# AwsGeek/thinvids

Measured on AMD Instinct MI355X. Metric: encoded frames/sec (whole node) at fixed PSNR, 1080p & 4K HEVC, 1/2/4/8 MI355X, higher is better.
Workload: dtype uint8 video / int32 integer transforms (bit-exact HEVC)

## Files before the change

csrc/core/capi.cpp:

```cpp
#include <cstring>
#include <exception>
#include <memory>
#include <string>
#include <vector>

#include "tv/av1_enc.h"
#include "tv/container.h"
#include "tv/cpu_encoder.h"
#include "tv/hevc_codec.h"
#include "tv/me_model.h"
#include "tv/sdh.h"
#include "tv/synth.h"
#include "tv/tb_frag.h"

using namespace tv;

namespace {
thread_local std::string g_err;
template <class F> int guard(F&& f) {
  try {
    f();
    return 0;
  } catch (const std::exception& e) {
    g_err = e.what();
    return -1;
  }
}
struct Bytes {
  std::vector<uint8_t> v;
};
}

extern "C" {

const char* tv_last_error() { return g_err.c_str(); }
int tv_core_version() { return 1; }

void* tv_bytes_new() { return new Bytes(); }
void tv_bytes_free(void* b) { delete static_cast<Bytes*>(b); }
size_t tv_bytes_size(void* b) { return static_cast<Bytes*>(b)->v.size(); }
const uint8_t* tv_bytes_data(void* b) { return static_cast<Bytes*>(b)->v.data(); }
void tv_bytes_clear(void* b) { static_cast<Bytes*>(b)->v.clear(); }

void tv_synth_frame(uint32_t seed, int t, int W, int H, uint8_t* y, uint8_t* u, uint8_t* v) {
  SynthFrameCtx ctx;
  synth_frame_ctx(seed, t, W, H, ctx);
  for (int c = 0; c < 3; ++c) {
    uint8_t* P = c == 0 ? y : (c == 1 ? u : v);
    const int w = c ? W / 2 : W, h = c ? H / 2 : H;
    for (int j = 0; j < h; ++j)
      for (int i = 0; i < w; ++i) P[(size_t)j * w + i] = (uint8_t)synth_sample_ctx(ctx, c, i, j);
  }
}

int tv_satd8x8(const int* d, int stride) { return satd8x8(d, stride); }

void* tv_cpu_encoder_new(int width, int height, int qp, int deblock, int range, int max_merge) {
  SeqConfig cfg;
  cfg.width = width;
  cfg.height = height;
  cfg.qp = qp;
  cfg.set_flags(deblock);
  cfg.max_merge_cand = max_merge;
  cfg.finalize();
  CpuEncoder* e = nullptr;
  guard([&] { e = new CpuEncoder(cfg, range); });
  return e;
}
void* tv_cpu_encoder_new_b(int width, int height, int qp, int deblock, int range, int max_merge, int mgop) {
  SeqConfig cfg;
  cfg.width = width;
  cfg.height = height;
  cfg.qp = qp;
  cfg.set_flags(deblock);
  cfg.max_merge_cand = max_merge;
  cfg.mgop = mgop;
  cfg.finalize();
  CpuEncoder* e = nullptr;
  guard([&] { e = new CpuEncoder(cfg, range); });
  return e;
}
int tv_cpu_encoder_begin_gop(void* e, int nframes, int* disp) {
  return guard([&] {
    auto* enc = static_cast<CpuEncoder*>(e);
    enc->begin_gop(nframes);
    for (size_t k = 0; k < enc->plan().pics.size(); ++k) disp[k] = enc->plan().pics[k].disp;
  });
}
int tv_gop_plan(int nframes, int mgop, int* disp, int* type, int* ref0, int* ref1, int* layer, int* info) {
  const GopPlan g = plan_gop(nframes, mgop);
  for (size_t k = 0; k < g.pics.size(); ++k) {
    disp[k] = g.pics[k].disp;
    type[k] = g.pics[k].type;
    ref0[k] = g.pics[k].ref[0];
    ref1[k] = g.pics[k].ref[1];
    layer[k] = g.pics[k].layer;
  }
  info[0] = g.dpb_size;
  info[1] = g.num_reorder;
  return (int)g.pics.size();
}
void* tv_cpu_encoder_new_crf(int width, int height, int qp, int deblock, int range, int max_merge, int crf) {
  SeqConfig cfg;
  cfg.width = width;
  cfg.height = height;
  cfg.qp = qp;
  cfg.set_flags(deblock);
  cfg.max_merge_cand = max_merge;
  cfg.crf = crf;
  cfg.finalize();
  CpuEncoder* e = nullptr;
  guard([&] { e = new CpuEncoder(cfg, range); });
  return e;
}
void tv_cpu_encoder_free(void* e) { delete static_cast<CpuEncoder*>(e); }
int tv_cpu_encoder_encode(void* e, const uint8_t* y, const uint8_t* u, const uint8_t* v, int sy,
                          int sc, int idr, int poc, void* out) {
  return guard([&] {
    const uint8_t* planes[3] = {y, u, v};
    const int strides[3] = {sy, sc, sc};
    static_cast<CpuEncoder*>(e)->encode_frame(planes, strides, idr != 0, poc, static_cast<Bytes*>(out)->v);
  });
}
int tv_cpu_encoder_encode_qp(void* e, const uint8_t* y, const uint8_t* u, const uint8_t* v, int sy, int sc, int idr,
                             int poc, int qp, void* out) {
  return guard([&] {
    const uint8_t* planes[3] = {y, u, v};
    const int strides[3] = {sy, sc, sc};
    static_cast<CpuEncoder*>(e)->encode_frame(planes, strides, idr != 0, poc, static_cast<Bytes*>(out)->v, qp);
  });
}
void tv_cpu_encoder_recon(void* e, uint8_t* y, uint8_t* u, uint8_t* v) {
  const Picture& p = static_cast<CpuEncoder*>(e)->recon();
  std::memcpy(y, p.y.data(), p.y.size());
// ... 201 lines not shown
```

csrc/gpu/k_frame.hip:

```cpp
#include <cstring>

#include "gpu_common.h"
#include "k_encode.h"
#include "tv/synth.h"

namespace tv {
namespace gpu {

struct VNoiseRow {
  int sh, sy;
  int32_t cy, cx;
  uint32_t seed;
  int a, b, c, d;
  __device__ void init(int32_t py16, int lp, uint32_t sd) {
    sh = lp + 4;
    seed = sd;
    cy = py16 >> sh;
    const int fy = (int)((py16 - (cy << sh)) << 8 >> sh);
    sy = (fy * fy * (768 - 2 * fy)) >> 16;
    cx = INT32_MIN;
  }
  __device__ int eval(int32_t px16) {
    const int32_t nx = px16 >> sh;
    if (nx != cx) {
      if (nx == cx + 1) {
        a = b;
        c = d;
      } else {
        a = synth_hash(nx, cy, seed) & 255;
        c = synth_hash(nx, cy + 1, seed) & 255;
      }
      b = synth_hash(nx + 1, cy, seed) & 255;
      d = synth_hash(nx + 1, cy + 1, seed) & 255;
      cx = nx;
    }
    const int fx = (int)((px16 - (cx << sh)) << 8 >> sh);
    const int sx = (fx * fx * (768 - 2 * fx)) >> 16;
    const int top = a * 256 + (b - a) * sx;
    const int bot = c * 256 + (d - c) * sx;
    return (top * 256 + (bot - top) * sy) >> 16;
  }
};

__device__ __forceinline__ int synth_objects(const SynthFrameCtx& f, int c, int xl, int yl, int v, unsigned rows) {
  for (; rows; rows &= rows - 1) {
    const int k = __builtin_ctz(rows);
    const SynthObject& o = f.obj[k];
    const int32_t rx16 = xl * 16 - f.ox[k], ry16 = yl * 16 - f.oy[k];
    if (rx16 < 0 || rx16 >= o.w * 16) continue;
    if (o.shape == 1) {
      const int64_t dx = 2 * (int64_t)rx16 - o.w * 16, dy = 2 * (int64_t)ry16 - o.h * 16;
      const int64_t ww = (int64_t)o.w * 16, hh = (int64_t)o.h * 16;
      if (dx * dx * hh * hh + dy * dy * ww * ww > ww * ww * hh * hh) continue;
    }
    if (c == 0) {
      v = 40 + ((synth_vnoise(rx16, ry16, 4, o.seed) * 3 + synth_vnoise(rx16, ry16, 2, o.seed + 5)) >> 2) * 3 / 4;
    } else {
      v = 64 + (int)(synth_hash(k, c, f.seed) & 127) + (synth_vnoise(rx16, ry16, 5, o.seed + c) >> 3);
    }
  }
  return v;
}

template <bool kTex>
__global__ void __launch_bounds__(256) k_synth(FrameSet src, Geo g, uint32_t seed, FrameIdx fi) {
  const int c = blockIdx.y, b = blockIdx.z;
  const int pw = c ? g.W / 2 : g.W, ph = c ? g.H / 2 : g.H;
  const int dw = c ? g.dw / 2 : g.dw, dh = c ? g.dh / 2 : g.dh;
  __shared__ SynthFrameCtx ctx;
  if (threadIdx.x == 0) synth_frame_ctx(seed, fi.t[b], g.dw, g.dh, ctx);
  __syncthreads();
  uint8_t* P = src.plane(c, b, g);
  const int s = c ? 1 : 0, pq = pw >> 2;
  constexpr bool tex = kTex;
  for (int i = blockIdx.x * blockDim.x + threadIdx.x; i < pq * ph; i += gridDim.x * blockDim.x) {
    const int y = i / pq, x0 = (i - y * pq) * 4;
    const int yc = tv_min(y, dh - 1), yl = yc << s;
    const int32_t by16 = yl * 16 + ctx.t * (tex ? 36 : 12);
    unsigned rows = 0;
#pragma unroll
    for (int k = 0; k < kSynthObjects; ++k) {
      const int32_t ry16 = yl * 16 - ctx.oy[k];
      rows |= (ry16 >= 0 && ry16 < ctx.obj[k].h * 16) ? 1u << k : 0u;
    }
    VNoiseRow n0, n1, n2, n3;
    if (c == 0) {
      n0.init(by16, 7, ctx.seed);
      n1.init(by16, 5, ctx.seed + 1);
      n2.init(by16, 3, ctx.seed + 2);
      if (tex) n3.init(by16, 1, ctx.seed + 3);
    } else {
      n0.init(by16, 8, ctx.seed + 10 * c);
    }
    uint32_t word = 0;
#pragma unroll
    for (int j = 0; j < 4; ++j) {
      const int xc = tv_min(x0 + j, dw - 1), xl = xc << s;
      const int32_t bx16 = xl * 16 + ctx.t * (tex ? 88 : 36);
      int v;
      if (c == 0 && tex)
        v = (n0.eval(bx16) * 3 + n1.eval(bx16) * 2 + n2.eval(bx16) * 2 + n3.eval(bx16)) >> 3;
      else if (c == 0)
        v = (n0.eval(bx16) * 5 + n1.eval(bx16) * 2 + n2.eval(bx16)) >> 3;
      else
        v = 96 + (n0.eval(bx16) >> 1);
      if (rows) v = synth_objects(ctx, c, xl, yl, v, rows);
      if (tex) {
        const uint32_t gr = synth_hash(xc + ctx.t * 7919, yc + c * 104729, ctx.seed ^ 0x5bd1e995u);
        v += c ? (int)(gr & 3) - 2 : (int)(gr & 7) - 4;
      }
      word |= (uint32_t)clip_pixel(v) << (8 * j);
    }
    *reinterpret_cast<uint32_t*>(P + (long)y * pw + x0) = word;
  }
}

__global__ void __launch_bounds__(256) k_sse(FrameSet a, FrameSet r, Geo g, unsigned long long* sse) {
  const int c = blockIdx.y, b = blockIdx.z;
  const int pw = c ? g.W / 2 : g.W;
  const int dw = c ? g.dw / 2 : g.dw, dh = c ? g.dh / 2 : g.dh;
  const uint8_t* A = a.plane(c, b, g);
  const uint8_t* R = r.plane(c, b, g);
  const int wq = (dw + 3) >> 2;
  unsigned s = 0;
  for (int i = blockIdx.x * blockDim.x + threadIdx.x; i < wq * dh; i += gridDim.x * blockDim.x) {
    const int y = i / wq, x = (i - y * wq) * 4;
    const uint32_t va = *reinterpret_cast<const uint32_t*>(A + (long)y * pw + x);
    const uint32_t vr = *reinterpret_cast<const uint32_t*>(R + (long)y * pw + x);
#pragma unroll
    for (int k = 0; k < 4; ++k) {
      const int d = (int)((va >> (8 * k)) & 255) - (int)((vr >> (8 * k)) & 255);
      s += (x + k < dw) ? (unsigned)(d * d) : 0u;
    }
  }
  unsigned long long t = s;
  for (int o = 32; o > 0; o >>= 1) t += __shfl_xor(t, o, 64);
  __shared__ unsigned long long part[4];
  if ((threadIdx.x & 63) == 0) part[threadIdx.x >> 6] = t;
  __syncthreads();
  if (threadIdx.x == 0) atomicAdd(sse + b * 3 + c, part[0] + part[1] + part[2] + part[3]);
}

typedef short tv_short2 __attribute__((ext_vector_type(2)));

__device__ constexpr uint32_t pack_taps4(int f, int k0) {
  return (uint32_t)(uint8_t)kLumaFilter[f][k0] | (uint32_t)(uint8_t)kLumaFilter[f][k0 + 1] << 8 |
         (uint32_t)(uint8_t)kLumaFilter[f][k0 + 2] << 16 | (uint32_t)(uint8_t)kLumaFilter[f][k0 + 3] << 24;
}
__device__ constexpr uint32_t pack_taps2(int f, int k0) {
  return (uint32_t)(uint16_t)kLumaFilter[f][k0] | (uint32_t)(uint16_t)kLumaFilter[f][k0 + 1] << 16;
}
__device__ __forceinline__ int dot4(uint32_t a, uint32_t b, int c) {
  return __builtin_amdgcn_sdot4((int)a, (int)b, c, false);
}
__device__ __forceinline__ int dot2(uint32_t a, uint32_t b, int c) {
  return __builtin_amdgcn_sdot2(__builtin_bit_cast(tv_short2, a), __builtin_bit_cast(tv_short2, b), c, false);
}
__device__ __forceinline__ uint32_t pack4_pixels(int v0, int v1, int v2, int v3) {
  return (uint32_t)clip_pixel(v0) | (uint32_t)clip_pixel(v1) << 8 | (uint32_t)clip_pixel(v2) << 16 |
         (uint32_t)clip_pixel(v3) << 24;
}

constexpr int kPhW = 10;
__global__ void __launch_bounds__(256) k_phase_planes(FrameSet ref, uint8_t* phase, Geo g) {
  const int tid = threadIdx.x;
  const int L = xcd_remap(blockIdx.x + gridDim.x * (blockIdx.y + gridDim.y * blockIdx.z),
                          gridDim.x * gridDim.y * gridDim.z);
  const int tpf = gridDim.x * gridDim.y, b = L / tpf, tyi = (L - b * tpf) / gridDim.x;
  const int tx0 = (L - b * tpf - tyi * gridDim.x) * 32 - 8, ty0 = tyi * 32 - 8;
  const uint8_t* R = ref.plane(0, b, g);
  __shared__ uint32_t raw[39][kPhW];
  __shared__ __align__(16) int16_t hf[3][39][32];
  for (int i = tid; i < 39 * kPhW; i += 256) {
    const int rr = i / kPhW, w = i - rr * kPhW;
    const uint8_t* row = R + (long)clip3(0, g.H - 1, ty0 - 3 + rr) * g.W;
    const int x = tx0 - 4 + 4 * w;
    uint32_t v;
    if (x >= 0 && x + 3 < g.W) {
      v = *reinterpret_cast<const uint32_t*>(row + x);
    } else {
      v = 0;
#pragma unroll
      for (int k = 0; k < 4; ++k) v |= (uint32_t)row[clip3(0, g.W - 1, x + k)] << (8 * k);
    }
    raw[rr][w] = v ^ 0x80808080u;
  }
  __syncthreads();
  for (int i = tid; i < 39 * 8; i += 256) {
    const int rr = i >> 3, c4 = i & 7;
    const uint32_t w0 = raw[rr][c4], w1 = raw[rr][c4 + 1], w2 = raw[rr][c4 + 2];
    int out[3][4];
#pragma unroll
    for (int j = 0; j < 4; ++j) {
      const uint32_t lo = j == 3 ? w1 : __builtin_amdgcn_alignbyte(w1, w0, j + 1);
      const uint32_t hi = j == 3 ? w2 : __builtin_amdgcn_alignbyte(w2, w1, j + 1);
#pragma unroll
      for (int f = 1; f < 4; ++f) out[f - 1][j] = dot4(lo, pack_taps4(f, 0), dot4(hi, pack_taps4(f, 4), 8192));
// ... 88 lines not shown
  uint8_t* U = rec.plane(1, b, g);
  uint8_t* V = rec.plane(2, b, g);
  const int W = g.W, H = g.H, Wc = W / 2;
  const int qpc = chroma_qp(qp, 0);
  const int nl = horizontal ? (H / 8 - 1) * (W / 4) : (W / 8 - 1) * (H / 4);
  const int nc = horizontal ? (H / 16 - 1) * (Wc / 4) : (W / 16 - 1) * (H / 8);
  auto ld = [](const uint8_t* p) { return *reinterpret_cast<const uint32_t*>(p); };
  auto st = [](uint8_t* p, uint32_t v) { *reinterpret_cast<uint32_t*>(p) = v; };
  for (int i = blockIdx.x * blockDim.x + threadIdx.x; i < nl + nc; i += gridDim.x * blockDim.x) {
    if (i < nl) {
      if (!horizontal) {
        const int x = 8 * (1 + i % (W / 8 - 1)), y = 4 * (i / (W / 8 - 1));
        const int bs = deblock_edge_bs(cl, in, cb, mv, g.w8, x - 1, y, x, y, dir, mv1, tu);
        if (bs) {
          uint32_t v[4][2];
#pragma unroll
          for (int k = 0; k < 4; ++k) {
            v[k][0] = ld(Y + (long)(y + k) * W + x - 4);
            v[k][1] = ld(Y + (long)(y + k) * W + x);
          }
          deblock_luma_edge4(reinterpret_cast<uint8_t*>(&v[0][1]), 1, 8, bs, qp);
#pragma unroll
          for (int k = 0; k < 4; ++k) {
            st(Y + (long)(y + k) * W + x - 4, v[k][0]);
            st(Y + (long)(y + k) * W + x, v[k][1]);
          }
        }
      } else {
        const int y = 8 * (1 + i % (H / 8 - 1)), x = 4 * (i / (H / 8 - 1));
        const int bs = deblock_edge_bs(cl, in, cb, mv, g.w8, x, y - 1, x, y, dir, mv1, tu);
        if (bs) {
          uint32_t v[8];
#pragma unroll
          for (int r = 0; r < 8; ++r) v[r] = ld(Y + (long)(y - 4 + r) * W + x);
          deblock_luma_edge4(reinterpret_cast<uint8_t*>(&v[4]), 4, 1, bs, qp);
#pragma unroll
          for (int r = 1; r < 7; ++r) st(Y + (long)(y - 4 + r) * W + x, v[r]);
        }
      }
    } else {
      const int j = i - nl;
      if (!horizontal) {
        const int xc = 8 * (1 + j % (W / 16 - 1)), yc = 4 * (j / (W / 16 - 1));
        const int bs = deblock_edge_bs(cl, in, cb, mv, g.w8, 2 * xc - 1, 2 * yc, 2 * xc, 2 * yc, dir, mv1, tu);
        if (bs == 2) {
#pragma unroll
          for (int pl = 0; pl < 2; ++pl) {
            uint8_t* P = pl ? V : U;
            uint32_t v[4][2];
#pragma unroll
            for (int k = 0; k < 4; ++k) {
              v[k][0] = ld(P + (long)(yc + k) * Wc + xc - 4);
              v[k][1] = ld(P + (long)(yc + k) * Wc + xc);
            }
            deblock_chroma_edge(reinterpret_cast<uint8_t*>(&v[0][1]), 1, 8, 4, qpc);
#pragma unroll
            for (int k = 0; k < 4; ++k) {
              st(P + (long)(yc + k) * Wc + xc - 4, v[k][0]);
              st(P + (long)(yc + k) * Wc + xc, v[k][1]);
            }
          }
        }
      } else {
        const int yc = 8 * (1 + j % (H / 16 - 1)), xc = 4 * (j / (H / 16 - 1));
        const int bs = deblock_edge_bs(cl, in, cb, mv, g.w8, 2 * xc, 2 * yc - 1, 2 * xc, 2 * yc, dir, mv1, tu);
        if (bs == 2) {
#pragma unroll
          for (int pl = 0; pl < 2; ++pl) {
            uint8_t* P = pl ? V : U;
            uint32_t v[4];
#pragma unroll
            for (int r = 0; r < 4; ++r) v[r] = ld(P + (long)(yc - 2 + r) * Wc + xc);
            deblock_chroma_edge(reinterpret_cast<uint8_t*>(&v[2]), 4, 1, 4, qpc);
            st(P + (long)(yc - 1) * Wc + xc, v[1]);
            st(P + (long)yc * Wc + xc, v[2]);
          }
        }
      }
    }
  }
}

void launch_synth(FrameSet src, const Geo& g, uint32_t seed, const FrameIdx& fi, int B, hipStream_t s) {
  dim3 grid((unsigned)tv_min(512, (int)((g.ysz + 1023) / 1024)), 3, B);
  if (synth_textured(seed))
    k_synth<true><<<grid, 256, 0, s>>>(src, g, seed, fi);
  else
    k_synth<false><<<grid, 256, 0, s>>>(src, g, seed, fi);
}
__global__ void __launch_bounds__(256) k_gather_frames(const uint8_t* frames, long seg_stride, FrameSet src, Geo g,
                                                       int B) {
  const long f16 = (g.ysz + 2 * g.csz) / 16, y16 = g.ysz / 16, c16 = g.csz / 16;
  for (long i = (long)blockIdx.x * 256 + threadIdx.x; i < B * f16; i += (long)gridDim.x * 256) {
    const int b = (int)(i / f16);
    const long r = i - b * f16;
    const uint4 v = reinterpret_cast<const uint4*>(frames + b * seg_stride)[r];
    uint4* d = r < y16 ? reinterpret_cast<uint4*>(src.y + b * g.ysz) + r
               : r < y16 + c16 ? reinterpret_cast<uint4*>(src.u + b * g.csz) + (r - y16)
                               : reinterpret_cast<uint4*>(src.v + b * g.csz) + (r - y16 - c16);
    *d = v;
  }
}
void launch_gather_frames(const uint8_t* frames, long seg_stride, FrameSet src, const Geo& g, int B, hipStream_t s) {
  const long n = B * (g.ysz + 2 * g.csz) / 16;
  k_gather_frames<<<(unsigned)tv_min(4096L, (n + 255) / 256), 256, 0, s>>>(frames, seg_stride, src, g, B);
}
struct QpArgs {
  int8_t q[64];
};
__global__ void __launch_bounds__(64) k_set_qp(int8_t* dst, QpArgs a, int n) {
  if ((int)threadIdx.x < n) dst[threadIdx.x] = a.q[threadIdx.x];
}
void launch_set_qp(int8_t* dst, const int8_t* host, int n, hipStream_t s) {
  for (int o = 0; o < n; o += 64) {
    QpArgs a;
    const int m = n - o < 64 ? n - o : 64;
    std::memcpy(a.q, host + o, (size_t)m);
    k_set_qp<<<1, 64, 0, s>>>(dst + o, a, m);
  }
}

void launch_sse(FrameSet a, FrameSet r, const Geo& g, unsigned long long* sse, int B, hipStream_t s) {
  dim3 grid((unsigned)tv_min(256, (int)((g.ysz / 4 + 4095) / 4096)), 3, B);
  k_sse<<<grid, 256, 0, s>>>(a, r, g, sse);
}
void launch_phase_planes(FrameSet ref, uint8_t* phase, const Geo& g, int B, hipStream_t s) {
  dim3 grid((g.W + 16 + 31) / 32, (g.H + 16 + 31) / 32, B);
  k_phase_planes<<<grid, 256, 0, s>>>(ref, phase, g);
}
constexpr int kSaoT = 34;
constexpr int kSaoTc = 18;
constexpr int kSaoP = kSaoT + 2, kSaoPc = kSaoTc + 2;
constexpr int kSaoTile = kSaoT * kSaoP + 2 * kSaoTc * kSaoPc;
constexpr int kSaoStage = (kSaoTile + 255) / 256;
__device__ __forceinline__ int sao_tix(int c, int row, int col) {
  return c == 0 ? row * kSaoP + col + 1 : kSaoT * kSaoP + (c - 1) * kSaoTc * kSaoPc + row * kSaoPc + col + 1;
}
typedef short sao_s2 __attribute__((ext_vector_type(2)));
__device__ __forceinline__ sao_s2 sao_pair(uint32_t w) { return __builtin_bit_cast(sao_s2, w); }
typedef unsigned short sao_u2 __attribute__((ext_vector_type(2)));
__device__ __forceinline__ sao_s2 sao_sign2(sao_s2 d) {
  const sao_s2 z = {0, 0};
  const sao_u2 f = {15, 15};
  return (d >> 15) | __builtin_bit_cast(sao_s2, __builtin_bit_cast(sao_u2, z - d) >> f);
}
__device__ __forceinline__ sao_s2 sao_relu2(sao_s2 e) { return e & ~(e >> 15); }
__device__ __forceinline__ sao_s2 sao_pkmax(sao_s2 a, sao_s2 b) {
  uint32_t r;
  asm("v_pk_max_i16 %0, %1, %2" : "=v"(r) : "v"(__builtin_bit_cast(uint32_t, a)), "v"(__builtin_bit_cast(uint32_t, b)));
  return sao_pair(r);
}
__device__ __forceinline__ sao_s2 sao_pkmin(sao_s2 a, sao_s2 b) {
  uint32_t r;
  asm("v_pk_min_i16 %0, %1, %2" : "=v"(r) : "v"(__builtin_bit_cast(uint32_t, a)), "v"(__builtin_bit_cast(uint32_t, b)));
  return sao_pair(r);
}

__device__ __forceinline__ void sao_tile_pos(int i, int& c, int& j) {
  c = i < kSaoT * kSaoT ? 0 : (i < kSaoT * kSaoT + kSaoTc * kSaoTc ? 1 : 2);
  j = c == 0 ? i : i - kSaoT * kSaoT - (c - 1) * kSaoTc * kSaoTc;
}

__global__ void __launch_bounds__(256) k_sao_decide(FrameSet src, FrameSet deb, FrameSet out, uint32_t* sao, Geo g,
                                                    const int8_t* qp, const RcTables* rc,
                                                    unsigned long long* sse) {
  const int tid = threadIdx.x, lane = tid & 63;
  int ctu, b;
  xcd_ctb(ctu, b);
  const long long lam16 = rc->sao_lam16[qp[b]];
  const int cx = ctu % g.wc, cy = ctu / g.wc;
  __shared__ SaoStats st[3];
// ... 321 lines not shown
```

thinvids_amd/_abi.py:

```python
import ctypes as C

i, l, ll, sz, ull, f32 = C.c_int, C.c_long, C.c_longlong, C.c_size_t, C.c_ulonglong, C.c_float
i32, i64, u32, vp, cstr = C.c_int32, C.c_int64, C.c_uint32, C.c_void_p, C.c_char_p
u8p, i8p, i16p, i32p, u32p = (C.POINTER(t) for t in (C.c_uint8, C.c_int8, C.c_int16, C.c_int32, C.c_uint32))
i64p, u64p, lp, llp, ullp, szp = (C.POINTER(t) for t in (C.c_int64, C.c_uint64, l, ll, ull, sz))
f64p, vpp = C.POINTER(C.c_double), C.POINTER(vp)


class SideTrack(C.Structure):
    _fields_ = [("kind", i32), ("codec", i32), ("timescale", i32), ("channels", i32), ("sample_rate", i32),
                ("bits", i32), ("is_default", i32), ("reserved", i32), ("lang", C.c_char * 4), ("mkv_codec_id", cstr),
                ("priv", vp), ("priv_size", C.c_uint64), ("path", cstr), ("data", vp), ("nsamples", i64),
                ("offsets", vp), ("sizes", vp), ("pts", vp), ("durs", vp)]


CORE = {
    "tv_core_build_hash": (cstr, []),
    "tv_last_error": (cstr, []),
    "tv_core_version": (i, []),
    "tv_bytes_new": (vp, []),
    "tv_bytes_free": (None, [vp]),
    "tv_bytes_size": (sz, [vp]),
    "tv_bytes_data": (vp, [vp]),
    "tv_bytes_clear": (None, [vp]),
    "tv_synth_frame": (None, [u32, i, i, i, u8p, u8p, u8p]),
    "tv_satd8x8": (i, [i32p, i]),
    "tv_cpu_encoder_new": (vp, [i] * 6),
    "tv_cpu_encoder_new_b": (vp, [i] * 7),
    "tv_cpu_encoder_new_crf": (vp, [i] * 7),
    "tv_cpu_encoder_free": (None, [vp]),
    "tv_cpu_encoder_begin_gop": (i, [vp, i, i32p]),
    "tv_gop_plan": (i, [i, i] + [i32p] * 6),
    "tv_cpu_encoder_encode": (i, [vp, u8p, u8p, u8p, i, i, i, i, vp]),
    "tv_cpu_encoder_encode_qp": (i, [vp, u8p, u8p, u8p, i, i, i, i, i, vp]),
    "tv_cpu_encoder_recon": (None, [vp, u8p, u8p, u8p]),
    "tv_cpu_encoder_decisions": (None, [vp, u8p, u8p, u8p, i16p, u8p]),
    "tv_cpu_encoder_levels": (None, [vp, i16p, i16p, i16p]),
    "tv_reconstruct_frame": (i, [i] * 4 + [u8p] * 9 + [i16p, u8p, i16p, i16p, i16p, u8p, u8p, u8p]),
    "tv_write_frame": (i, [i] * 7 + [u8p, u8p, u8p, i16p, u8p, i16p, i16p, i16p, vp]),
    "tv_mv_rate": (None, [i32p, i32p, i, i32p, i32p]),
    "tv_av1_mv_comp_bits": (None, [i32p, i, i32p]),
    "tv_tb_frag_expand": (i, [i, i32p]),
    "tv_quant_levels": (None, [i32p, i, i, i, i32p, i32p]),
    "tv_sdh_deltas": (None, [i32p, i, i, i, i, i32p, i32p]),
    "tv_hevc_spec_table": (i, [cstr, i32p, i]),
    "tv_decoder_new": (vp, []),
    "tv_decoder_free": (None, [vp]),
    "tv_decoder_decode": (i, [vp, u8p, sz]),
    "tv_decoder_decode_range": (i, [vp, u8p, sz, i, i]),
    "tv_decoder_info": (None, [vp] + [i32p] * 5),
    "tv_decoder_frame": (i, [vp, i, i, u8p, u8p, u8p]),
    "tv_hevc_scale_mv": (None, [i, i, i, i, i32p]),
    "tv_hevc_display_offsets": (i, [u8p, sz, i32p, i]),
    "tv_hevc_probe": (i, [u8p, sz] + [i32p] * 4),
    "tv_mux_mp4": (i, [u8p, sz, i, i, i, i, vp]),
    "tv_mux_mp4_file": (i, [vpp, szp, i, i, i, i, i, cstr, ullp]),
    "tv_mux_file": (i, [vpp, szp, i, i, i, i, i, C.POINTER(SideTrack), i, i, cstr, ullp]),
    "tv_side_track_size": (sz, []),
    "tv_demux_mp4": (i, [u8p, sz] + [i32p] * 5 + [vp]),
    "tv_mp4s_open": (vp, [cstr, i, i, i, i, ull]),
    "tv_mp4s_append": (i, [vp, u8p, sz]),
    "tv_mp4s_close": (i, [vp, ullp]),
    "tv_mp4s_abort": (None, [vp]),
    "tv_mp4s_last_error": (cstr, []),
    "tv_io_last_error": (cstr, []),
    "tv_pread_parallel": (ll, [cstr, ll, ll, vp, i]),
    "tv_readahead": (i, [cstr, ll, ll]),
    "tv_av1c_last_error": (cstr, []),
    "tv_av1c_qlookup": (i, [i, i]),
    "tv_av1c_golden_encode": (i, [i, i, i, u8p, i, i32p, vp, i64p, u8p, u32p, u32p, i16p, i16p, i16p, i32p, i8p,
                                  i32p]),
    "tv_av1c_golden_encode_tools": (i, [i, i, i, u8p, i, i32p, i, vp, i64p, u8p, u32p, u32p, i16p, i16p, i16p, i32p,
                                        i8p, i32p, u8p]),
    "tv_av1c_ib_accept": (i, [u8p, i, i, u8p]),
    "tv_av1c_cfl_decide": (i, [u8p, u8p, u8p, i, i, i, i, i32p]),
    "tv_av1c_decode": (i, [u8p, sz, i, u8p, i32p, i32p]),
    "tv_av1c_probe": (i, [u8p, sz, i32p, i32p]),
    "tv_av1c_state_new": (vp, []),
    "tv_av1c_state_free": (None, [vp]),
    "tv_av1c_write_tu": (i, [vp, i, i, i32p, u32p, u32p, i16p, i16p, i16p, i8p, i32p, i, i, vp]),
    "tv_av1_last_error": (cstr, []),
    "tv_av1_cdef_find_dirs": (None, [u8p, i, i, u8p, i32p]),
    "tv_av1_cdef_search": (None, [u8p, u8p, i, i, i, u8p, i32p, i, i, u64p]),
    "tv_av1_cdef_apply": (None, [u8p, i, i, i, u8p, i32p, i, i, i8p, u8p]),
    "tv_av1_wiener_apply": (None, [u8p, i, i, i32p, u8p]),
    "tv_av1_wiener_stats": (None, [u8p, u8p, i, i, i, i32p, i64p]),
    "tv_av1_sgr_apply": (None, [u8p, i, i, i32p, u8p]),
    "tv_av1_sgr_stats": (None, [u8p, u8p, i, i, i, i64p]),
    "tv_av1_sgr_filter_planes": (None, [u8p, i, i, i, i32p, i32p]),
    "tv_av1_deblock": (i, [u8p, i, i, i, u32p, i, u8p]),
    "tv_av1_rc_roundtrip": (i, [i32p, i32p, i32p, i, i, i, vp, i32p]),
    "tv_av1_txfm_ref": (i, [i16p, i16p, i, i, i, i, i]),
    "tv_av1_txfm_basis": (i, [i, i, i32p]),
    "tv_mpeg2_last_error": (cstr, []),
    "tv_mpeg2_encode": (i, [i32p, i, i, u8p, vp, i64p, i32p, u8p]),
    "tv_mpeg2_probe": (i, [u8p, sz, i32p]),
    "tv_mpeg2_raps": (i, [u8p, sz, i64p, i64p, i32p, i32p, i]),
    "tv_mpeg2_decode": (i, [u8p, sz, i64, i64, i32, i32, i32, u8p, i32p, i64p]),
    "tv_mpeg2_table": (i, [i, i32p, i32p, i32p, i]),
    "tv_mpeg2_stat_name": (cstr, [i]),
    "tv_mpeg2_num_stats": (i, []),
}

GPU = {
    "tv_gpu_build_hash": (cstr, []),
    "tv_gpu_last_error": (cstr, []),
    "tv_gpu_device_count": (i, []),
    "tv_engine_new_b": (vp, [i] * 7 + [u32, i, i, i, i, i]),
# ... 62 lines not shown
```

Baseline: 10730.

## Rewrite synthetic frame kernel as tiled lattice/top-row shared-memory evaluation

The GPU synth kernel now works on 256x32 tiles. Each block builds the value-noise lattice and the horizontally interpolated rows in LDS once, and threads only do the vertical blend, so hashes are no longer recomputed per pixel. Per-frame object context is computed on the host and passed as kernel arguments instead of by one thread per block. A CPU tiled reference and a shared header are added for bit-exactness checks. Synthetic frame generation is probably a small part of the end-to-end encode throughput, and the extra syncs and LDS use could limit occupancy.

```diff
diff --git a/csrc/core/capi.cpp b/csrc/core/capi.cpp
--- a/csrc/core/capi.cpp
+++ b/csrc/core/capi.cpp
@@ -11,6 +11,7 @@
 #include "tv/me_model.h"
 #include "tv/sdh.h"
 #include "tv/synth.h"
+#include "tv/synth_tile.h"
 #include "tv/tb_frag.h"
 
 using namespace tv;
@@ -29,6 +30,79 @@
 struct Bytes {
   std::vector<uint8_t> v;
 };
+
+struct TileOctave {
+  int nx = 0;
+  std::vector<uint8_t> lat;
+  std::vector<uint16_t> top;
+  std::vector<int> cy, sy;
+  void build(int lp, uint32_t seed, const std::vector<int32_t>& px, const std::vector<int32_t>& py) {
+    const SynthWin w = synth_win(lp, seed, px.front(), px.back(), py.front(), py.back());
+    nx = (int)px.size();
+    lat.resize((size_t)w.npx * w.npy);
+    for (int r = 0; r < w.npy; ++r)
+      for (int i = 0; i < w.npx; ++i) lat[(size_t)r * w.npx + i] = (uint8_t)synth_win_lattice(w, i, r);
+    top.resize((size_t)w.npy * nx);
+    for (int x = 0; x < nx; ++x) {
+      int ci, sx;
+      synth_axis(px[x], w.sh, w.cx0, ci, sx);
+      for (int r = 0; r < w.npy; ++r)
+        top[(size_t)r * nx + x] = (uint16_t)synth_top(lat[(size_t)r * w.npx + ci], lat[(size_t)r * w.npx + ci + 1], sx);
+    }
+    cy.resize(py.size());
+    sy.resize(py.size());
+    for (size_t y = 0; y < py.size(); ++y) synth_axis(py[y], w.sh, w.cy0, cy[y], sy[y]);
+  }
+  int at(int x, int y) const {
+    const uint16_t* t = &top[(size_t)cy[y] * nx + x];
+    return synth_rows(t[0], t[nx], sy[y]);
+  }
+};
+
+void synth_tile_fill(const SynthFrameCtx& f, int c, int x0, int y0, int nx, int ny, int pw, uint8_t* P) {
+  const int s = c ? 1 : 0, dw = c ? f.W / 2 : f.W, dh = c ? f.H / 2 : f.H;
+  const bool tex = synth_textured(f.seed);
+  std::vector<int32_t> px(nx), py(ny), qx(nx), qy(ny);
+  for (int x = 0; x < nx; ++x) px[x] = synth_tile_pos(x0 + x, dw, s);
+  for (int y = 0; y < ny; ++y) py[y] = synth_tile_pos(y0 + y, dh, s);
+  std::vector<int> v((size_t)nx * ny);
+  TileOctave oct[4];
+  for (int x = 0; x < nx; ++x) qx[x] = px[x] + f.t * synth_pan_x(tex);
+  for (int y = 0; y < ny; ++y) qy[y] = py[y] + f.t * synth_pan_y(tex);
+  const int nb = synth_bg_octaves(c, tex);
+  for (int i = 0; i < nb; ++i) oct[i].build(synth_bg_lp(c, i), synth_bg_seed(f.seed, c, i), qx, qy);
+  for (int y = 0; y < ny; ++y)
+    for (int x = 0; x < nx; ++x) {
+      int n[4] = {0, 0, 0, 0};
+      for (int i = 0; i < nb; ++i) n[i] = oct[i].at(x, y);
+      v[(size_t)y * nx + x] = synth_bg_mix(c, tex, n);
+    }
+  for (int k = 0; k < kSynthObjects; ++k) {
+    const SynthObject& o = f.obj[k];
+    int32_t xlo, xhi, ylo, yhi;
+    synth_obj_range(px.front(), px.back(), f.ox[k], o.w, xlo, xhi);
+    synth_obj_range(py.front(), py.back(), f.oy[k], o.h, ylo, yhi);
+    if (xlo > xhi || ylo > yhi) continue;
+    for (int x = 0; x < nx; ++x) qx[x] = clip3(xlo, xhi, px[x] - f.ox[k]);
+    for (int y = 0; y < ny; ++y) qy[y] = clip3(ylo, yhi, py[y] - f.oy[k]);
+    const int no = synth_obj_octaves(c), base = synth_obj_base(f.seed, k, c);
+    for (int i = 0; i < no; ++i) oct[i].build(synth_obj_lp(c, i), synth_obj_seed(o, c, i), qx, qy);
+    for (int y = 0; y < ny; ++y)
+      for (int x = 0; x < nx; ++x) {
+        const int32_t rx16 = px[x] - f.ox[k], ry16 = py[y] - f.oy[k];
+        if (rx16 != qx[x] || ry16 != qy[y] || synth_cover_col(o, rx16) > synth_cover_row(o, ry16)) continue;
+        int n[2] = {0, 0};
+        for (int i = 0; i < no; ++i) n[i] = oct[i].at(x, y);
+        v[(size_t)y * nx + x] = synth_obj_mix(c, base, n);
+      }
+  }
+  for (int y = 0; y < ny; ++y)
+    for (int x = 0; x < nx; ++x) {
+      int r = v[(size_t)y * nx + x];
+      if (tex) r += synth_grain(f.seed, f.t, c, tv_min(x0 + x, dw - 1), tv_min(y0 + y, dh - 1));
+      P[(size_t)(y0 + y) * pw + x0 + x] = (uint8_t)clip_pixel(r);
+    }
+}
 }
 
 extern "C" {
@@ -50,6 +124,20 @@
     const int w = c ? W / 2 : W, h = c ? H / 2 : H;
     for (int j = 0; j < h; ++j)
       for (int i = 0; i < w; ++i) P[(size_t)j * w + i] = (uint8_t)synth_sample_ctx(ctx, c, i, j);
+  }
+}
+
+void tv_synth_frame_tiled(uint32_t seed, int t, int W, int H, int tile_w, int tile_h, uint8_t* y, uint8_t* u,
+                          uint8_t* v) {
+  SynthFrameCtx ctx;
+  synth_frame_ctx(seed, t, W, H, ctx);
+  const int cw = (W + kCtb - 1) / kCtb * kCtb, ch = (H + kCtb - 1) / kCtb * kCtb;
+  for (int c = 0; c < 3; ++c) {
+    uint8_t* P = c == 0 ? y : (c == 1 ? u : v);
+    const int pw = c ? cw / 2 : cw, ph = c ? ch / 2 : ch;
+    for (int y0 = 0; y0 < ph; y0 += tile_h)
+      for (int x0 = 0; x0 < pw; x0 += tile_w)
+        synth_tile_fill(ctx, c, x0, y0, tv_min(tile_w, pw - x0), tv_min(tile_h, ph - y0), pw, P);
   }
 }
 
diff --git a/csrc/gpu/k_frame.hip b/csrc/gpu/k_frame.hip
--- a/csrc/gpu/k_frame.hip
+++ b/csrc/gpu/k_frame.hip
@@ -3,116 +3,192 @@
 #include "gpu_common.h"
 #include "k_encode.h"
 #include "tv/synth.h"
+#include "tv/synth_tile.h"
 
 namespace tv {
 namespace gpu {
 
-struct VNoiseRow {
-  int sh, sy;
-  int32_t cy, cx;
-  uint32_t seed;
-  int a, b, c, d;
-  __device__ void init(int32_t py16, int lp, uint32_t sd) {
-    sh = lp + 4;
-    seed = sd;
-    cy = py16 >> sh;
-    const int fy = (int)((py16 - (cy << sh)) << 8 >> sh);
-    sy = (fy * fy * (768 - 2 * fy)) >> 16;
-    cx = INT32_MIN;
-  }
-  __device__ int eval(int32_t px16) {
-    const int32_t nx = px16 >> sh;
-    if (nx != cx) {
-      if (nx == cx + 1) {
-        a = b;
-        c = d;
-      } else {
-        a = synth_hash(nx, cy, seed) & 255;
-        c = synth_hash(nx, cy + 1, seed) & 255;
-      }
-      b = synth_hash(nx + 1, cy, seed) & 255;
-      d = synth_hash(nx + 1, cy + 1, seed) & 255;
-      cx = nx;
-    }
-    const int fx = (int)((px16 - (cx << sh)) << 8 >> sh);
-    const int sx = (fx * fx * (768 - 2 * fx)) >> 16;
-    const int top = a * 256 + (b - a) * sx;
-    const int bot = c * 256 + (d - c) * sx;
-    return (top * 256 + (bot - top) * sy) >> 16;
-  }
+constexpr int kSynTW = kSynthTileW, kSynTH = kSynthTileH, kSynRows = kSynTH / 4;
+static_assert(kSynTW == 256 && kSynTH % 4 == 0, "a wave of 4-sample items spans the tile; 4 waves share its rows");
+
+struct SynthArgs {
+  SynthObject obj[kSynthObjects];
+  int32_t t[kMaxBatch];
+  int32_t ox[kMaxBatch][kSynthObjects], oy[kMaxBatch][kSynthObjects];
 };
-
-__device__ __forceinline__ int synth_objects(const SynthFrameCtx& f, int c, int xl, int yl, int v, unsigned rows) {
-  for (; rows; rows &= rows - 1) {
-    const int k = __builtin_ctz(rows);
-    const SynthObject& o = f.obj[k];
-    const int32_t rx16 = xl * 16 - f.ox[k], ry16 = yl * 16 - f.oy[k];
-    if (rx16 < 0 || rx16 >= o.w * 16) continue;
-    if (o.shape == 1) {
-      const int64_t dx = 2 * (int64_t)rx16 - o.w * 16, dy = 2 * (int64_t)ry16 - o.h * 16;
-      const int64_t ww = (int64_t)o.w * 16, hh = (int64_t)o.h * 16;
-      if (dx * dx * hh * hh + dy * dy * ww * ww > ww * ww * hh * hh) continue;
-    }
-    if (c == 0) {
-      v = 40 + ((synth_vnoise(rx16, ry16, 4, o.seed) * 3 + synth_vnoise(rx16, ry16, 2, o.seed + 5)) >> 2) * 3 / 4;
-    } else {
-      v = 64 + (int)(synth_hash(k, c, f.seed) & 127) + (synth_vnoise(rx16, ry16, 5, o.seed + c) >> 3);
-    }
-  }
-  return v;
+static_assert(sizeof(SynthArgs) + sizeof(Geo) + sizeof(FrameSet) + 16 <= 4096, "kernel arguments are limited to 4 KB");
+
+constexpr int kSynSpanX = (kSynTW - 1) * 16, kSynSpanY = (kSynTH - 1) * 16;
+constexpr int syn_max(int a, int b) { return a > b ? a : b; }
+constexpr int syn_pts(int lp, int s) { return synth_win_max(kSynSpanX << s, lp) * synth_win_max(kSynSpanY << s, lp); }
+constexpr int syn_rows(int lp, int s) { return synth_win_max(kSynSpanY << s, lp); }
+constexpr int syn_lat_size(bool tex) {
+  return syn_max(syn_max(syn_pts(7, 0) + syn_pts(5, 0) + syn_pts(3, 0) + (tex ? syn_pts(1, 0) : 0), syn_pts(4, 0) + syn_pts(2, 0)),
+                 syn_max(syn_pts(8, 1), syn_pts(5, 1)));
+}
+constexpr int syn_top_rows(bool tex) {
+  return syn_max(syn_max(syn_rows(7, 0) + syn_rows(5, 0) + syn_rows(3, 0) + (tex ? syn_rows(1, 0) : 0), syn_rows(4, 0) + syn_rows(2, 0)),
+                 syn_max(syn_rows(8, 1), syn_rows(5, 1)));
+}
+
+__device__ __forceinline__ void syn_lattice(const SynthWin& w, uint8_t* lat, int wave, int lane) {
+  for (int r = wave; r < w.npy; r += 4)
+    for (int i = lane; i < w.npx; i += 64) lat[r * w.npx + i] = (uint8_t)synth_win_lattice(w, i, r);
+}
+__device__ __forceinline__ void syn_top(const SynthWin& w, const uint8_t* lat, uint16_t* top, int col, int32_t p16) {
+  int ci, sx;
+  synth_axis(p16, w.sh, w.cx0, ci, sx);
+  for (int r = 0; r < w.npy; ++r)
+    top[r * kSynTW + col] = (uint16_t)synth_top(lat[r * w.npx + ci], lat[r * w.npx + ci + 1], sx);
+}
+__device__ __forceinline__ void syn_eval(const SynthWin& w, const uint16_t* top, int x, int32_t p16, int n[4]) {
+  int cy, sy;
+  synth_axis(p16, w.sh, w.cy0, cy, sy);
+  const uint2 a = *reinterpret_cast<const uint2*>(top + cy * kSynTW + x);
+  const uint2 b = *reinterpret_cast<const uint2*>(top + (cy + 1) * kSynTW + x);
+  n[0] = synth_rows((int)(a.x & 0xffff), (int)(b.x & 0xffff), sy);
+  n[1] = synth_rows((int)(a.x >> 16), (int)(b.x >> 16), sy);
+  n[2] = synth_rows((int)(a.y & 0xffff), (int)(b.y & 0xffff), sy);
+  n[3] = synth_rows((int)(a.y >> 16), (int)(b.y >> 16), sy);
+}
+
+template <bool kTex, bool kChroma>
+__device__ __forceinline__ void syn_tile(uint16_t* top, uint8_t* lat, FrameSet src, const Geo& g, uint32_t seed,
+                                         const SynthArgs& a, int c, int x0, int y0) {
+  constexpr int kBg = kChroma ? 1 : (kTex ? 4 : 3), kOb = kChroma ? 1 : 2, s = kChroma ? 1 : 0;
+  __builtin_assume(kChroma ? c != 0 : c == 0);
+  const int b = blockIdx.y;
+  const int pw = g.W >> s, ph = g.H >> s, dw = g.dw >> s, dh = g.dh >> s;
+  const int t = a.t[b];
+  const int tid = threadIdx.x, lane = tid & 63, wave = __builtin_amdgcn_readfirstlane(tid >> 6);
+  const int32_t tx0 = synth_tile_pos(x0, dw, s), tx1 = synth_tile_pos(x0 + kSynTW - 1, dw, s);
+  const int32_t ty0 = synth_tile_pos(y0, dh, s), ty1 = synth_tile_pos(y0 + kSynTH - 1, dh, s);
+  const int32_t colp = synth_tile_pos(x0 + tid, dw, s);
+  const int x = 4 * lane, yw = y0 + wave * kSynRows;
+  int32_t sp[4];
+#pragma unroll
+  for (int j = 0; j < 4; ++j) sp[j] = synth_tile_pos(x0 + x + j, dw, s);
+
+  SynthWin w[kBg];
+  int lat0[kBg], row0[kBg];
+  const int panx = t * synth_pan_x(kTex), pany = t * synth_pan_y(kTex);
+  {
+    int lo = 0, ro = 0;
+#pragma unroll
+    for (int i = 0; i < kBg; ++i) {
+      w[i] = synth_win(synth_bg_lp(c, i), synth_bg_seed(seed, c, i), tx0 + panx, tx1 + panx, ty0 + pany, ty1 + pany);
+      lat0[i] = lo;
+      row0[i] = ro;
+      syn_lattice(w[i], lat + lo, wave, lane);
+      lo += w[i].npx * w[i].npy;
+      ro += w[i].npy;
+    }
+  }
+  __syncthreads();
+#pragma unroll
+  for (int i = 0; i < kBg; ++i) syn_top(w[i], lat + lat0[i], top + row0[i] * kSynTW, tid, colp + panx);
+  __syncthreads();
+  uint32_t word[kSynRows];
+#pragma unroll
+  for (int j = 0; j < kSynRows; ++j) {
+    const int32_t py = synth_tile_pos(yw + j, dh, s) + pany;
+    int n[4][4] = {};
+#pragma unroll
+    for (int i = 0; i < kBg; ++i) syn_eval(w[i], top + row0[i] * kSynTW, x, py, n[i]);
+    word[j] = 0;
+#pragma unroll
+    for (int q = 0; q < 4; ++q) {
+      const int m[4] = {n[0][q], n[1][q], n[2][q], n[3][q]};
+      word[j] |= (uint32_t)synth_bg_mix(c, kTex, m) << (8 * q);
+    }
+  }
+
+  for (int k = 0; k < kSynthObjects; ++k) {
+    const SynthObject& o = a.obj[k];
+    const int32_t ox = a.ox[b][k], oy = a.oy[b][k];
+    int32_t xlo, xhi, ylo, yhi;
+    synth_obj_range(tx0, tx1, ox, o.w, xlo, xhi);
+    synth_obj_range(ty0, ty1, oy, o.h, ylo, yhi);
+    if (xlo > xhi || ylo > yhi) continue;
+    const int base = synth_obj_base(seed, k, c);
+    SynthWin wo[kOb];
+    int olat[kOb], orow[kOb];
+    __syncthreads();
+    {
+      int lo = 0, ro = 0;
+#pragma unroll
+      for (int i = 0; i < kOb; ++i) {
+        wo[i] = synth_win(synth_obj_lp(c, i), synth_obj_seed(o, c, i), xlo, xhi, ylo, yhi);
+        olat[i] = lo;
+        orow[i] = ro;
+        syn_lattice(wo[i], lat + lo, wave, lane);
+        lo += wo[i].npx * wo[i].npy;
+        ro += wo[i].npy;
+      }
+    }
+    __syncthreads();
+#pragma unroll
+    for (int i = 0; i < kOb; ++i) syn_top(wo[i], lat + olat[i], top + orow[i] * kSynTW, tid, clip3(xlo, xhi, colp - ox));
+    __syncthreads();
+    int64_t cover[4];
+#pragma unroll
+    for (int q = 0; q < 4; ++q) {
+      const int32_t rx16 = sp[q] - ox;
+      cover[q] = rx16 < xlo || rx16 > xhi ? INT64_MAX : synth_cover_col(o, rx16);
+    }
+#pragma unroll
+    for (int j = 0; j < kSynRows; ++j) {
+      const int32_t ry16 = synth_tile_pos(yw + j, dh, s) - oy;
+      if (ry16 < ylo || ry16 > yhi) continue;
+      const int64_t cover_row = synth_cover_row(o, ry16);
+      int n[2][4] = {};
+#pragma unroll
+      for (int i = 0; i < kOb; ++i) syn_eval(wo[i], top + orow[i] * kSynTW, x, ry16, n[i]);
+#pragma unroll
+      for (int q = 0; q < 4; ++q) {
+        if (cover[q] > cover_row) continue;
+        const int m[2] = {n[0][q], n[1][q]};
+        word[j] = (word[j] & ~(0xffu << (8 * q))) | (uint32_t)synth_obj_mix(c, base, m) << (8 * q);
+      }
+    }
+  }
+
+  if (x0 + x >= pw) return;
+  uint8_t* P = src.plane(c, b, g);
+#pragma unroll
+  for (int j = 0; j < kSynRows; ++j) {
+    const int y = yw + j;
+    if (y >= ph) break;
+    uint32_t out = word[j];
+    if (kTex) {
+      const int yc = tv_min(y, dh - 1);
+      out = 0;
+#pragma unroll
+      for (int q = 0; q < 4; ++q) {
+        const int v = (int)((word[j] >> (8 * q)) & 255) + synth_grain(seed, t, c, tv_min(x0 + x + q, dw - 1), yc);
+        out |= (uint32_t)clip_pixel(v) << (8 * q);
+      }
+    }
+    *reinterpret_cast<uint32_t*>(P + (long)y * pw + x0 + x) = out;
+  }
 }
 
 template <bool kTex>
-__global__ void __launch_bounds__(256) k_synth(FrameSet src, Geo g, uint32_t seed, FrameIdx fi) {
-  const int c = blockIdx.y, b = blockIdx.z;
-  const int pw = c ? g.W / 2 : g.W, ph = c ? g.H / 2 : g.H;
-  const int dw = c ? g.dw / 2 : g.dw, dh = c ? g.dh / 2 : g.dh;
-  __shared__ SynthFrameCtx ctx;
-  if (threadIdx.x == 0) synth_frame_ctx(seed, fi.t[b], g.dw, g.dh, ctx);
-  __syncthreads();
-  uint8_t* P = src.plane(c, b, g);
-  const int s = c ? 1 : 0, pq = pw >> 2;
-  constexpr bool tex = kTex;
-  for (int i = blockIdx.x * blockDim.x + threadIdx.x; i < pq * ph; i += gridDim.x * blockDim.x) {
-    const int y = i / pq, x0 = (i - y * pq) * 4;
-    const int yc = tv_min(y, dh - 1), yl = yc << s;
-    const int32_t by16 = yl * 16 + ctx.t * (tex ? 36 : 12);
-    unsigned rows = 0;
-#pragma unroll
-    for (int k = 0; k < kSynthObjects; ++k) {
-      const int32_t ry16 = yl * 16 - ctx.oy[k];
-      rows |= (ry16 >= 0 && ry16 < ctx.obj[k].h * 16) ? 1u << k : 0u;
-    }
-    VNoiseRow n0, n1, n2, n3;
-    if (c == 0) {
-      n0.init(by16, 7, ctx.seed);
-      n1.init(by16, 5, ctx.seed + 1);
-      n2.init(by16, 3, ctx.seed + 2);
-      if (tex) n3.init(by16, 1, ctx.seed + 3);
-    } else {
-      n0.init(by16, 8, ctx.seed + 10 * c);
-    }
-    uint32_t word = 0;
-#pragma unroll
-    for (int j = 0; j < 4; ++j) {
-      const int xc = tv_min(x0 + j, dw - 1), xl = xc << s;
-      const int32_t bx16 = xl * 16 + ctx.t * (tex ? 88 : 36);
-      int v;
-      if (c == 0 && tex)
-        v = (n0.eval(bx16) * 3 + n1.eval(bx16) * 2 + n2.eval(bx16) * 2 + n3.eval(bx16)) >> 3;
-      else if (c == 0)
-        v = (n0.eval(bx16) * 5 + n1.eval(bx16) * 2 + n2.eval(bx16)) >> 3;
-      else
-        v = 96 + (n0.eval(bx16) >> 1);
-      if (rows) v = synth_objects(ctx, c, xl, yl, v, rows);
-      if (tex) {
-        const uint32_t gr = synth_hash(xc + ctx.t * 7919, yc + c * 104729, ctx.seed ^ 0x5bd1e995u);
-        v += c ? (int)(gr & 3) - 2 : (int)(gr & 7) - 4;
-      }
-      word |= (uint32_t)clip_pixel(v) << (8 * j);
-    }
-    *reinterpret_cast<uint32_t*>(P + (long)y * pw + x0) = word;
-  }
+__global__ void __launch_bounds__(256) k_synth(FrameSet src, Geo g, uint32_t seed, SynthArgs a) {
+  __shared__ __attribute__((aligned(8))) uint16_t top[syn_top_rows(kTex) * kSynTW];
+  __shared__ uint8_t lat[syn_lat_size(kTex)];
+  const int nlx = (g.W + kSynTW - 1) / kSynTW, ncx = (g.W / 2 + kSynTW - 1) / kSynTW;
+  const int nl = nlx * ((g.H + kSynTH - 1) / kSynTH), nc = ncx * ((g.H / 2 + kSynTH - 1) / kSynTH);
+  int id = blockIdx.x, c = 0;
+  if (id >= nl) {
+    c = id >= nl + nc ? 2 : 1;
+    id -= nl + (c - 1) * nc;
+  }
+  const int ntx = c ? ncx : nlx, ty = id / ntx, x0 = (id - ty * ntx) * kSynTW, y0 = ty * kSynTH;
+  if (c)
+    syn_tile<kTex, true>(top, lat, src, g, seed, a, c, x0, y0);
+  else
+    syn_tile<kTex, false>(top, lat, src, g, seed, a, 0, x0, y0);
 }
 
 __global__ void __launch_bounds__(256) k_sse(FrameSet a, FrameSet r, Geo g, unsigned long long* sse) {
@@ -367,11 +443,22 @@
 }
 
 void launch_synth(FrameSet src, const Geo& g, uint32_t seed, const FrameIdx& fi, int B, hipStream_t s) {
-  dim3 grid((unsigned)tv_min(512, (int)((g.ysz + 1023) / 1024)), 3, B);
+  SynthArgs a;
+  std::memset(&a, 0, sizeof a);
+  SynthFrameCtx f;
+  for (int b = 0; b < B; ++b) {
+    synth_frame_ctx(seed, fi.t[b], g.dw, g.dh, f);
+    a.t[b] = f.t;
+    std::memcpy(a.ox[b], f.ox, sizeof f.ox);
+    std::memcpy(a.oy[b], f.oy, sizeof f.oy);
+  }
+  if (B > 0) std::memcpy(a.obj, f.obj, sizeof f.obj);
+  auto tiles = [](int w, int h) { return ((w + kSynTW - 1) / kSynTW) * ((h + kSynTH - 1) / kSynTH); };
+  dim3 grid((unsigned)(tiles(g.W, g.H) + 2 * tiles(g.W / 2, g.H / 2)), (unsigned)B);
   if (synth_textured(seed))
-    k_synth<true><<<grid, 256, 0, s>>>(src, g, seed, fi);
+    k_synth<true><<<grid, 256, 0, s>>>(src, g, seed, a);
   else
-    k_synth<false><<<grid, 256, 0, s>>>(src, g, seed, fi);
+    k_synth<false><<<grid, 256, 0, s>>>(src, g, seed, a);
 }
 __global__ void __launch_bounds__(256) k_gather_frames(const uint8_t* frames, long seg_stride, FrameSet src, Geo g,
                                                        int B) {
diff --git a/csrc/include/tv/synth_tile.h b/csrc/include/tv/synth_tile.h
--- /dev/null
+++ b/csrc/include/tv/synth_tile.h
@@ -0,0 +1,78 @@
+#pragma once
+#include <cstdint>
+
+#include "synth.h"
+
+namespace tv {
+
+constexpr int kSynthTileW = 256, kSynthTileH = 32;
+
+TV_HD int32_t synth_tile_pos(int i, int d, int s) { return (int32_t)((tv_min(i, d - 1) << s) * 16); }
+
+struct SynthWin {
+  int sh;
+  uint32_t seed;
+  int32_t cx0, cy0;
+  int npx, npy;
+};
+TV_HD SynthWin synth_win(int lp, uint32_t seed, int32_t px_lo, int32_t px_hi, int32_t py_lo, int32_t py_hi) {
+  SynthWin w;
+  w.sh = lp + 4;
+  w.seed = seed;
+  w.cx0 = px_lo >> w.sh;
+  w.cy0 = py_lo >> w.sh;
+  w.npx = (px_hi >> w.sh) - w.cx0 + 2;
+  w.npy = (py_hi >> w.sh) - w.cy0 + 2;
+  return w;
+}
+constexpr int synth_win_max(int span16, int lp) { return (span16 >> (lp + 4)) + 3; }
+
+TV_HD int synth_win_lattice(const SynthWin& w, int i, int r) {
+  return (int)(synth_hash(w.cx0 + i, w.cy0 + r, w.seed) & 255);
+}
+TV_HD void synth_axis(int32_t p16, int sh, int32_t c0, int& ci, int& sw) {
+  const int32_t cc = p16 >> sh;
+  const int f = (int)((p16 - (cc << sh)) << 8 >> sh);
+  sw = (f * f * (768 - 2 * f)) >> 16;
+  ci = (int)(cc - c0);
+}
+TV_HD int synth_top(int a, int b, int sx) { return a * 256 + (b - a) * sx; }
+TV_HD int synth_rows(int top, int bot, int sy) { return (top * 256 + (bot - top) * sy) >> 16; }
+
+TV_HD int synth_pan_x(bool tex) { return tex ? 88 : 36; }
+TV_HD int synth_pan_y(bool tex) { return tex ? 36 : 12; }
+TV_HD int synth_bg_octaves(int c, bool tex) { return c ? 1 : (tex ? 4 : 3); }
+TV_HD int synth_bg_lp(int c, int i) { return c ? 8 : 7 - 2 * i; }
+TV_HD uint32_t synth_bg_seed(uint32_t seed, int c, int i) { return c ? seed + 10 * c : seed + i; }
+TV_HD int synth_bg_mix(int c, bool tex, const int n[4]) {
+  if (c) return 96 + (n[0] >> 1);
+  return tex ? (n[0] * 3 + n[1] * 2 + n[2] * 2 + n[3]) >> 3 : (n[0] * 5 + n[1] * 2 + n[2]) >> 3;
+}
+TV_HD int synth_obj_octaves(int c) { return c ? 1 : 2; }
+TV_HD int synth_obj_lp(int c, int i) { return c ? 5 : 4 - 2 * i; }
+TV_HD uint32_t synth_obj_seed(const SynthObject& o, int c, int i) { return c ? o.seed + c : o.seed + 5 * i; }
+TV_HD int synth_obj_mix(int c, int base, const int n[2]) {
+  return c ? 64 + base + (n[0] >> 3) : 40 + ((n[0] * 3 + n[1]) >> 2) * 3 / 4;
+}
+TV_HD int synth_obj_base(uint32_t seed, int k, int c) { return (int)(synth_hash(k, c, seed) & 127); }
+TV_HD int64_t synth_cover_col(const SynthObject& o, int32_t rx16) {
+  if (o.shape != 1) return 0;
+  const int64_t dx = 2 * (int64_t)rx16 - o.w * 16, hh = (int64_t)o.h * 16;
+  return dx * dx * hh * hh;
+}
+TV_HD int64_t synth_cover_row(const SynthObject& o, int32_t ry16) {
+  if (o.shape != 1) return 0;
+  const int64_t dy = 2 * (int64_t)ry16 - o.h * 16, ww = (int64_t)o.w * 16, hh = (int64_t)o.h * 16;
+  return ww * ww * hh * hh - dy * dy * ww * ww;
+}
+TV_HD int synth_grain(uint32_t seed, int t, int c, int xc, int yc) {
+  const uint32_t g = synth_hash(xc + t * 7919, yc + c * 104729, seed ^ 0x5bd1e995u);
+  return c ? (int)(g & 3) - 2 : (int)(g & 7) - 4;
+}
+
+TV_HD void synth_obj_range(int32_t p_lo, int32_t p_hi, int32_t o16, int extent, int32_t& lo, int32_t& hi) {
+  lo = tv_max(p_lo - o16, 0);
+  hi = tv_min(p_hi - o16, extent * 16 - 1);
+}
+
+}
diff --git a/thinvids_amd/_abi.py b/thinvids_amd/_abi.py
--- a/thinvids_amd/_abi.py
+++ b/thinvids_amd/_abi.py
@@ -24,6 +24,7 @@
     "tv_bytes_data": (vp, [vp]),
     "tv_bytes_clear": (None, [vp]),
     "tv_synth_frame": (None, [u32, i, i, i, u8p, u8p, u8p]),
+    "tv_synth_frame_tiled": (None, [u32, i, i, i, i, i, u8p, u8p, u8p]),
     "tv_satd8x8": (i, [i32p, i]),
     "tv_cpu_encoder_new": (vp, [i] * 6),
     "tv_cpu_encoder_new_b": (vp, [i] * 7),
```

Result: faster. 11880, median of 6 (+10.7%).
